# PJLab-ADG/DetZero

Measured on AMD Instinct MI355X. Metric: LiDAR frames/sec (160k pts, 0.1m voxels), higher is better.
Workload: dtype f32 as f16 pairs (hi+lo, 22-bit significand; 3 f16 MFMA per product, f32 accumulate)

## Files before the change

### detzero_amd/det_modules.py

```python
import contextlib
import os
from functools import partial

import numpy as np
import torch
import torch.nn as nn

from . import ops
from .lib import DetZeroHipError

PACKED_TABLES = bool(os.environ.get('DZ_TUNE_PACKED_TABLES'))

K3, S1, P1 = (3, 3, 3), (1, 1, 1), (1, 1, 1)


def _inference_only(module):
    if module.training:
        raise DetZeroHipError('%s: only the inference path is implemented on the HIP backend '
                              '(call .eval()); training is out of scope' % type(module).__name__)


def fold_bn(bn, conv_bias=None):
    w = bn.weight.detach().double()
    b = bn.bias.detach().double()
# ... 526 lines not shown


def bordered_zeros(name, shape, dev):
    ws = _WORKSPACE[0]
    if ws is None:
        return torch.zeros(shape, dtype=torch.float32, device=dev)
    key = (name, tuple(shape), str(dev))
    buf = ws.get(key)
    if buf is None:
        buf = ws[key] = torch.zeros(shape, dtype=torch.float32, device=dev)
    return buf


def nchw_to_padded_nhwc(x, pad=1):
    b, c, h, w = x.shape
    out = x.new_zeros((b, h + 2 * pad, w + 2 * pad, c))
    out[:, pad:pad + h, pad:pad + w, :] = x.permute(0, 2, 3, 1)
    return out


def _recode(img, enc, math, e_src=0, e_dst=0):
    if ops.storage_math(enc) == ops.storage_math(math) and e_src == e_dst:
        return img
    plain = ops.pair16_to_f32(img, enc) if enc else img
    if e_src != e_dst:
        plain = plain * (2.0 ** (e_dst - e_src))
    return ops.pair16_from_f32(plain, math=math) if math else plain


SKIP_EMPTY_TILES = os.environ.get('DZ_TUNE_SKIP_EMPTY_TILES', '1') != '0'
SPARSE_BEV_INPUT = os.environ.get('DZ_TUNE_SPARSE_BEV', '1') != '0'
FIRST_BLOCK_WIDE_GROUPS = os.environ.get('DZ_TUNE_FIRST_BLOCK_WIDE', '1') != '0'
FUSED_DEBLOCK_PHASES = os.environ.get('DZ_TUNE_DEBLOCK_PHASES', '1') != '0'


def conv_layer(inp, in_shape, w, scale, shift, relu, out, out_shape, *, cin, in_cstride, in_coff=0, ksize=3,
               stride=1, in_off=0, out_cstride, out_coff=0, out_s=1, out_d=(0, 0), groups=1, cout_pad=None,
               g_cout=None, g_ooff=None, ho=None, wo=None, batch=1, math=0, out_f32=False, phase_groups=False, in_rowidx=None,
               in_row_channels=0, in_rows=0, in_tiles=None):
    if cout_pad is None:
        cout_pad = w.shape[-2] if math else w.shape[-1]
    ops.conv2d(dict(
        inp=inp.data_ptr(), out=out.data_ptr(), w=w.data_ptr(),
        scale=scale.data_ptr() if scale is not None else None,
        shift=shift.data_ptr() if shift is not None else None,
        batch=batch, ho=ho, wo=wo, in_hp=in_shape[0], in_wp=in_shape[1], in_cstride=in_cstride, in_coff=in_coff,
        cin=cin, kh=ksize, kw=ksize, stride=stride, in_off=in_off,
        out_hp=out_shape[0], out_wp=out_shape[1], out_cstride=out_cstride, out_coff=out_coff,
        out_sy=out_s, out_sx=out_s, out_dy=out_d[0], out_dx=out_d[1],
        groups=groups, cout_pad=cout_pad,
        g_cout=g_cout if g_cout is not None else [cout_pad], g_ooff=g_ooff if g_ooff is not None else [0],
        relu=1 if relu else 0, phase_groups=1 if phase_groups else 0,
        in_rowidx=in_rowidx.data_ptr() if in_rowidx is not None else None, in_row_channels=int(in_row_channels), in_rows=int(in_rows),
        in_tiles=in_tiles.data_ptr() if in_tiles is not None else None),
        math=math, out_f32=out_f32, tiles=in_tiles)


class BaseBEVBackbone(_Cached):

    def __init__(self, model_cfg, input_channels):
        super().__init__()
        self.model_cfg = model_cfg
        layer_nums = list(model_cfg.LAYER_NUMS)
        layer_strides = list(model_cfg.LAYER_STRIDES)
        num_filters = list(model_cfg.NUM_FILTERS)
        upsample_strides = list(model_cfg.UPSAMPLE_STRIDES)
        num_upsample_filters = list(model_cfg.NUM_UPSAMPLE_FILTERS)
        assert len(layer_nums) == len(layer_strides) == len(num_filters) == len(upsample_strides)
        c_in_list = [input_channels, *num_filters[:-1]]
        self.blocks = nn.ModuleList()
        self.deblocks = nn.ModuleList()
        for idx in range(len(layer_nums)):
            cur = [nn.ZeroPad2d(1),
                   nn.Conv2d(c_in_list[idx], num_filters[idx], kernel_size=3, stride=layer_strides[idx], padding=0, bias=False),
                   nn.BatchNorm2d(num_filters[idx], eps=1e-3, momentum=0.01), nn.ReLU()]
            for _ in range(layer_nums[idx]):
                cur.extend([nn.Conv2d(num_filters[idx], num_filters[idx], kernel_size=3, padding=1, bias=False),
                            nn.BatchNorm2d(num_filters[idx], eps=1e-3, momentum=0.01), nn.ReLU()])
            self.blocks.append(nn.Sequential(*cur))
            s = upsample_strides[idx]
            if not (isinstance(s, int) and s >= 1):
                raise DetZeroHipError('BaseBEVBackbone: only integer UPSAMPLE_STRIDES >= 1 are supported')
            self.deblocks.append(nn.Sequential(
                nn.ConvTranspose2d(num_filters[idx], num_upsample_filters[idx], s, stride=s, bias=False),
                nn.BatchNorm2d(num_upsample_filters[idx], eps=1e-3, momentum=0.01), nn.ReLU()))
        self.num_bev_features = sum(num_upsample_filters)
        self.layer_strides, self.upsample_strides = layer_strides, upsample_strides
        self.num_filters, self.num_upsample_filters = num_filters, num_upsample_filters
# ... 75 lines not shown
                if not getattr(self, '_warned_capture_nl1', False):
                    self._warned_capture_nl1 = True
                    import warnings
                    warnings.warn('BaseBEVBackbone: graph capture of a %d-frame pass without an eager pass of the same size before it - empty tiles '
                                  'are skipped at the first layer only (run one eager pass first to skip them in all six)' % batch)
            tiles = ops.bev_tile_list(sparse_in[1], xh, xw, nl)
            zero = self._zero_response(lvl, xh, xw, sparse_in[0].shape[1], dev, batch) if nl > 1 else None
        for ci, cv in enumerate(convs):
            s = cv['stride']
            oh, ow = (xh + 2 - 3) // s + 1, (xw + 2 - 3) // s + 1
            if bufs is None:
                bufs = [bordered_zeros('bev2d.l%d.%d' % (li, k), (batch, oh + 2, ow + 2, cv['cout']), dev) for k in range(2)]
            y = out_last if (out_last is not None and ci == len(convs) - 1) else bufs[ci % 2]
            if sparse_in is not None and li == 0 and ci == 0:
                rows, ridx = sparse_in
                wz, scz, shz = self._p(cv, e_in, e_mid, key='w_zmajor')
                conv_layer(rows, (xh + 2, xw + 2), wz, scz, shz, True, y, (oh + 2, ow + 2),
                           cin=cv['cin'], in_cstride=xc, ksize=3, stride=s, in_off=0, out_cstride=cv['cout'],
                           out_d=(1, 1), ho=oh, wo=ow, batch=batch, math=self.math, in_rowidx=ridx, in_row_channels=rows.shape[1],
                           in_rows=rows.shape[0], in_tiles=tiles[0] if tiles is not None else None)
                if tiles is not None:
                    ops.bev_fill_empty_tiles(tiles[0], batch, oh, ow, shz, True, cv['cout'], y, self.math)
            else:
                tl = tiles[ci] if (tiles is not None and ci < tiles.shape[0]) else None
                wc, scc, shc = self._p(cv, e_in if (li == 0 and ci == 0) else e_mid, e_mid)
                conv_layer(x, (xh + 2, xw + 2), wc, scc, shc, True, y, (oh + 2, ow + 2),
                           cin=cv['cin'], in_cstride=xc, ksize=3, stride=s, in_off=0, out_cstride=cv['cout'],
                           out_d=(1, 1), ho=oh, wo=ow, batch=batch, math=self.math, in_tiles=tl)
                if tl is not None:
                    ops.bev_fill_empty_tiles(tl, batch, oh, ow, shc, True, cv['cout'], y, self.math, zero_resp=zero[ci])
            x, xh, xw, xc = y, oh, ow, cv['cout']
        return x, xh, xw, xc

    def _level_deblock(self, lvl, x, xh, xw, xc, concat, coff, h, w, batch):
        de = lvl['de']
        s = de['s']
        ctot = self.num_bev_features
        e_mid = self._e('spatial_features_2d')
        if xh * s != h or xw * s != w:
            raise DetZeroHipError('BaseBEVBackbone: deblock output %dx%d does not match %dx%d' % (xh * s, xw * s, h, w))
        if self.math and 1 < s * s <= 8 and FUSED_DEBLOCK_PHASES:
            conv_layer(x, (xh + 2, xw + 2), *self._p(de, e_mid, e_mid, key='w_phases'), True, concat,
                       (h + 2, w + 2), cin=de['cin'], in_cstride=xc, ksize=1, stride=1, in_off=1,
                       out_cstride=ctot, out_coff=coff, out_s=s, out_d=(1, 1), ho=xh, wo=xw, batch=batch, math=self.math,
                       groups=s * s, g_cout=[de['cout']] * (s * s), g_ooff=[0] * (s * s), phase_groups=True)
            return coff + de['cout']
        for dy in range(s):
            for dx in range(s):
                conv_layer(x, (xh + 2, xw + 2), *self._p(de['phases'][dy][dx], e_mid, e_mid, scale=de['scale'], shift=de['shift']), True, concat,
                           (h + 2, w + 2), cin=de['cin'], in_cstride=xc, ksize=1, stride=1, in_off=1,
                           out_cstride=ctot, out_coff=coff, out_s=s, out_d=(dy + 1, dx + 1), ho=xh, wo=xw,
                           batch=batch, math=self.math)
        return coff + de['cout']

    def run(self, bev, batch, sparse_in=None):
        plan = self.plan()
        if sparse_in is not None:
            rows, ridx = sparse_in
            dev = rows.device
            h, w = ridx.shape[1] - 2, ridx.shape[2] - 2
        else:
            dev = bev.device
            h, w = bev.shape[1] - 2, bev.shape[2] - 2
        concat = bordered_zeros('bev2d.concat', (batch, h + 2, w + 2, self.num_bev_features), dev)
        x, xh, xw, xc = bev, h, w, (bev.shape[3] if sparse_in is None else 2 * rows.shape[1])
        coff = 0
        for li, lvl in enumerate(plan):
            x, xh, xw, xc = self._level_convs(li, lvl, x, xh, xw, xc, batch, dev, sparse_in=sparse_in if li == 0 else None)
            coff = self._level_deblock(lvl, x, xh, xw, xc, concat, coff, h, w, batch)
        return concat

    def grouped_fits(self, nb, h, w):
        plan = self.plan()
        xh, xw, worst = h, w, 0
        for lvl in plan:
            s = lvl['convs'][0]['stride']
            xh, xw = (xh + 2 - 3) // s + 1, (xw + 2 - 3) // s + 1
            worst = max(worst, (xh + 2) * (xw + 2) * lvl['convs'][-1]['cout'] * 4)
        return nb * worst < 2 ** 31

    def run_grouped(self, nb, group, consume, bev=None, sparse_in=None):
        plan = self.plan()
        if sparse_in is not None:
            rows, ridx = sparse_in
            dev = rows.device
            h, w = ridx.shape[1] - 2, ridx.shape[2] - 2
            cin0 = 2 * rows.shape[1]
        else:
            dev = bev.device
            h, w = bev.shape[1] - 2, bev.shape[2] - 2
            cin0 = bev.shape[3]
        l0 = plan[0]
        s0 = l0['convs'][0]['stride']
        h0, w0 = (h + 2 - 3) // s0 + 1, (w + 2 - 3) // s0 + 1
        c0 = l0['convs'][-1]['cout']
        if len(l0['convs']) < 2:
            raise DetZeroHipError('BaseBEVBackbone.run_grouped: the first block needs at least two convolutions')
        x0_all = bordered_zeros('bev2d.x0_all', (nb, h0 + 2, w0 + 2, c0), dev)
        widest = max([cin0] + [cv['cout'] for cv in l0['convs']])
        group1 = max(group, min(nb, (2 ** 31 - 1) // ((h + 2) * (w + 2) * widest * 4))) if FIRST_BLOCK_WIDE_GROUPS else group
        for g0 in range(0, nb, group1):
            ng = min(group1, nb - g0)
            sp = (rows, ridx[g0:g0 + ng]) if sparse_in is not None else None
            self._level_convs(0, l0, None if sp is not None else bev[g0:g0 + ng], h, w, cin0, ng, dev, sparse_in=sp, out_last=x0_all[g0:g0 + ng])
        outs = [(x0_all, h0, w0, c0)]
        x, xh, xw, xc = outs[0]
        for li in range(1, len(plan)):
            x, xh, xw, xc = self._level_convs(li, plan[li], x, xh, xw, xc, nb, dev)
            outs.append((x, xh, xw, xc))
        for g0 in range(0, nb, group):
            ng = min(group, nb - g0)
            concat = bordered_zeros('bev2d.concat', (ng, h + 2, w + 2, self.num_bev_features), dev)
            coff = 0
            for lvl, (x, xh, xw, xc) in zip(plan, outs):
                coff = self._level_deblock(lvl, x[g0:g0 + ng], xh, xw, xc, concat, coff, h, w, ng)
            consume(concat, g0, ng)

    def forward(self, data_dict):
        _inference_only(self)
        with torch.no_grad():
            bev = data_dict.get('_nhwc_spatial_features', None)
            enc = data_dict.get('_nhwc_math', 0)
            e_src = int(data_dict.get('_nhwc_exp', 0) or 0)
            if bev is None:
                bev, enc = nchw_to_padded_nhwc(data_dict['spatial_features'].float()), 0
                e_src = 0
            bev = _recode(bev, enc, self.math, e_src, self._e('encoded'))
            concat = self.run(bev, bev.shape[0])
        e_out = self._e('spatial_features_2d')
        data_dict['_nhwc_spatial_features_2d'] = concat
        data_dict['_nhwc_math'] = self.math
        data_dict['_nhwc_exp'] = e_out
        plain = ops.pair16_to_f32(concat, self.math) if self.math else concat
        if e_out:
            plain = plain * (2.0 ** -e_out)
        data_dict['spatial_features_2d'] = plain[:, 1:-1, 1:-1, :].permute(0, 3, 1, 2)
        return data_dict


class SeparateHead(nn.Module):

    def __init__(self, input_channels, sep_head_dict, init_bias=-2.19, use_bias=False):
        super().__init__()
        self.sep_head_dict = sep_head_dict
        for cur_name in self.sep_head_dict:
            output_channels = self.sep_head_dict[cur_name]['out_channels']
            num_conv = self.sep_head_dict[cur_name]['num_conv']
            fc_list = []
# ... 230 lines not shown
```

### detzero_amd/lib.py

```python
import ctypes
import os

import torch

_HERE = os.path.dirname(os.path.abspath(__file__))
LIB_PATH = os.path.join(_HERE, 'libdetzero_hip.so')


ERR_INVALID, ERR_WORKSPACE, ERR_HIP, ERR_UNSUPPORTED = -1, -2, -3, -4


class DetZeroHipError(RuntimeError):
    pass


c_int, c_float, c_size_t, c_void_p, c_double = ctypes.c_int, ctypes.c_float, ctypes.c_size_t, ctypes.c_void_p, ctypes.c_double
_I3 = c_int * 3
_F3 = c_float * 3
_F6 = c_float * 6
_I8 = c_int * 8


class Conv2dDesc(ctypes.Structure):
    _fields_ = [
# ... 75 lines not shown
    'dz_spconv_forward_split_packed': (c_int, [c_void_p, c_int, c_int, c_void_p, c_void_p, c_int, c_void_p, c_void_p, c_void_p,
                                               c_void_p, c_void_p, c_int, c_void_p, c_int, c_int, c_void_p]),
    'dz_spconv_tile_rows': (c_int, []),
    'dz_spconv_tile_info_words': (c_int, []),
    'dz_spconv_tile_table_entries': (c_int, []),
    'dz_build_tiles_halo_stride': (c_size_t, [c_int]),
    'dz_build_tiles': (c_int, [c_void_p, c_int, c_int, c_void_p, c_void_p, c_void_p, c_void_p, c_void_p, c_void_p]),
    'dz_spconv_tiles_forward': (c_int, [c_void_p, c_int, c_int, c_void_p, c_void_p, c_void_p, c_void_p, c_int, c_int, c_void_p, c_void_p,
                                        c_void_p, c_void_p, c_void_p, c_int, c_void_p, c_int, c_int, c_void_p]),
    'dz_spconv_tiles_variant': (ctypes.c_char_p, [c_int, c_int]),
    'dz_spconv_x_tile_rows': (c_int, [c_int, c_int]),
    'dz_spconv_x_window_rows': (c_int, [c_int, c_int]),
    'dz_spconv_x_windows_words': (c_size_t, [c_int, c_int]),
    'dz_spconv_x_windows': (c_int, [c_void_p, c_int, c_void_p, c_int, c_void_p, c_void_p, c_void_p, c_void_p]),
    'dz_build_neighbors_packed_x': (c_int, [c_void_p, c_void_p, c_int, c_void_p, c_void_p, c_int, c_int, c_int, c_int, c_void_p, c_void_p, c_int,
                                            c_void_p, c_void_p, c_void_p, c_void_p]),
    'dz_spconv_forward_split_x': (c_int, [c_void_p, c_int, c_int, c_void_p, c_void_p, c_void_p, c_int, c_int, c_void_p, c_void_p, c_void_p, c_void_p,
                                          c_void_p, c_int, c_void_p, c_int, c_int, c_void_p]),
    'dz_spconv_x_variant': (ctypes.c_char_p, [c_int, c_int]),
    'dz_spconv_forward_x_f32': (c_int, [c_void_p, c_int, c_int, c_void_p, c_void_p, c_void_p, c_int, c_int, c_void_p, c_void_p, c_void_p, c_void_p,
                                        c_void_p, c_int, c_void_p, c_int, c_void_p]),
    'dz_spconv_x_f32_window_rows': (c_int, [c_int, c_int]),
    'dz_spconv_x_f32_variant': (ctypes.c_char_p, [c_int, c_int]),
    'dz_bev_tile_list_words': (c_size_t, [c_int, c_int, c_int]),
    'dz_bev_tile_list': (c_int, [c_void_p, c_int, c_int, c_int, c_int, c_int, c_int, c_void_p, c_void_p, c_void_p]),
    'dz_bev_fill_empty_tiles': (c_int, [c_void_p, c_int, c_int, c_int, c_void_p, c_int, c_int, c_void_p, c_int, c_int, c_int, c_int, c_void_p, c_int, c_void_p]),
    'dz_bev_row_index': (c_int, [c_void_p, c_void_p, c_int, c_int, c_int, c_int, c_int, c_int, c_int, c_void_p, c_void_p]),
    'dz_sparse_to_bev_split': (c_int, [c_void_p, c_void_p, c_void_p, c_int, c_int, c_int, c_int, c_int, c_int, c_void_p,
                                       c_void_p]),
    'dz_sparse_to_bev_split_dense': (c_int, [c_void_p, c_int, c_void_p, c_void_p, c_int, c_int, c_int, c_int, c_int, c_int, c_int, c_void_p,
                                             c_void_p]),
    'dz_conv2d_forward_split': (c_int, [ctypes.POINTER(Conv2dDesc), c_int, c_int, c_void_p]),
    'dz_conv2d_variant_split': (ctypes.c_char_p, [ctypes.POINTER(Conv2dDesc), c_int]),
    'dz_spconv_variant_split': (ctypes.c_char_p, [c_int, c_int]),
    'dz_spconv_variant_split_arm': (ctypes.c_char_p, [c_int, c_int, c_int, c_int, c_size_t]),
    'dz_spconv_variant_split_packed': (ctypes.c_char_p, [c_int, c_int]),
    'dz_xattn_folded_supported': (c_int, [c_int, c_int, c_int]),
    'dz_xattn_folded_workspace_bytes': (ctypes.c_size_t, [c_int, c_int]),
    'dz_xattn_folded': (c_int, [c_void_p] * 6 + [c_int] * 5 + [ctypes.c_float, c_void_p, ctypes.c_size_t, c_void_p, c_void_p]),
    'dz_roi_bev_features': (c_int, [c_void_p, c_int, c_void_p, ctypes.c_long, ctypes.c_long, c_int, c_int, c_int] + [ctypes.c_float] * 4 + [c_int, c_void_p, c_void_p]),
    'dz_linear_splitk_workspace_bytes': (ctypes.c_size_t, [c_int, c_int, c_int]),
    'dz_linear_forward_splitk': (c_int, [c_void_p, c_int, c_int, c_int, c_void_p, c_int, c_int, c_void_p, c_void_p, c_int, c_void_p, c_int, c_int, c_void_p,
                                         ctypes.c_size_t, c_void_p]),
    'dz_mha_core_split': (c_int, [c_void_p, c_void_p, c_void_p, c_void_p, c_int, c_int, c_int, c_int, ctypes.c_float, c_void_p, c_int, c_void_p]),
    'dz_pdv_sa_pool_supported': (c_int, [c_int] * 7),
    'dz_pdv_sa_pool': (c_int, [c_void_p, c_int, c_int, c_void_p, c_void_p, c_int, c_void_p, c_void_p, c_int, c_void_p, c_void_p, c_int,
                               c_void_p, c_int, c_void_p, c_void_p, c_int, c_void_p, c_int, c_void_p, c_void_p, c_int, c_int, c_void_p, c_void_p]),
    'dz_pdv_encoder_front': (c_int, [c_void_p, c_int, c_void_p, c_void_p, ctypes.c_long] + [c_void_p] * 9 + [c_int, c_void_p]),
    'dz_pdv_encoder_back': (c_int, [c_void_p, c_void_p, c_void_p, c_void_p, ctypes.c_long, c_void_p, c_void_p, c_void_p, c_void_p, c_float, c_void_p, c_void_p,
                                    c_void_p, c_void_p, c_void_p, c_void_p, c_float, c_void_p, c_int, c_int, c_void_p]),
    'dz_self_attention_split_supported': (c_int, [c_int, c_int]),
    'dz_self_attention_split': (c_int, [c_void_p, c_void_p, c_void_p, c_int, c_int, c_int, c_void_p, c_int, c_void_p]),
    'dz_pdv_sa_pool_split_supported': (c_int, [c_int] * 7),
    'dz_pdv_sa_pool_split': (c_int, [c_void_p, c_int, c_int, c_void_p, c_void_p, ctypes.c_long, c_int, c_void_p, c_void_p, c_int, c_void_p, c_void_p, c_int,
                                     c_void_p, c_int, c_void_p, c_void_p, c_int, c_void_p, c_int, c_void_p, c_void_p, c_int, c_int, c_int, c_void_p, c_int, c_void_p]),
    'dz_mlp_chain_forward': (c_int, [c_void_p, ctypes.c_long, c_void_p, c_void_p, c_void_p, c_void_p, c_int, c_int] + [c_void_p] * 10 + [c_int, c_void_p]),
    'dz_pointnet3_forward': (c_int, [c_void_p, ctypes.c_long] + [c_void_p] * 9 + [c_int, c_int, c_void_p, c_void_p, c_int, c_int, c_void_p]),
    'dz_centerhead_decode_workspace_bytes': (c_size_t, [c_int] * 4),
    'dz_centerhead_decode': (c_int, [c_void_p, c_int, c_int, c_int, c_int, c_int, c_float, c_void_p, c_void_p,
                                     c_void_p, c_int, c_int, c_void_p, c_void_p, c_void_p, c_void_p, c_void_p,
                                     c_size_t, c_void_p]),
    'dz_nms_workspace_bytes': (c_size_t, [c_int]),
    'dz_nms_rotated': (c_int, [c_void_p, c_void_p, c_int, c_float, c_int, c_void_p, c_void_p, c_void_p, c_size_t,
                               c_void_p]),
    'dz_nms_rotated_batched': (c_int, [c_void_p, c_void_p, c_int, c_int, c_float, c_int, c_void_p, c_void_p, c_void_p, c_size_t,
                                       c_void_p]),
# ... 92 lines not shown
```

### detzero_amd/ops.py

```python
import ctypes
import os

import numpy as np
import torch

from . import lib as L


def _dev():
    return torch.device('cuda', torch.cuda.current_device())


def _ws(nbytes):
    return torch.empty((max(int(nbytes), 256),), dtype=torch.uint8, device=_dev())


def grid_size_of(pc_range, voxel_size):
    r = np.asarray(pc_range, dtype=np.float32)
    return np.round((r[3:6] - r[0:3]) / np.array(voxel_size)).astype(np.int64)


def voxelize_hard_nosync(points, pc_range, voxel_size, max_points, max_voxels, xy_range_mask=False):
    lib = L.load()
    L.require_cuda(points)
# ... 474 lines not shown
    for _ in red:
        up = up.unsqueeze(-2)
    return w.float() * up, down


def level_rows_f32(rows, level, math=0):
    plain = pair16_to_f32(rows, math) if math else rows
    e = int(getattr(level, 'act_exp', 0) or 0)
    return plain * (2.0 ** -e) if e else plain


def pair16_from_f32(x, c_dst=None, math=1):
    lib = L.load()
    L.require_cuda(x)
    x = x.contiguous()
    c = x.shape[-1]
    c_dst = c if c_dst is None else c_dst
    rows = x.numel() // c
    out = torch.empty((*x.shape[:-1], c_dst), dtype=torch.float32, device=x.device)
    L.check(lib.dz_pair16_from_f32(L.ptr(x), rows, c, c_dst, storage_math(math), L.ptr(out), L.stream()), 'dz_pair16_from_f32')
    return out


def pair16_to_f32(x, math=1):
    lib = L.load()
    L.require_cuda(x)
    x = x.contiguous()
    c = x.shape[-1]
    out = torch.empty_like(x)
    L.check(lib.dz_pair16_to_f32(L.ptr(x), x.numel() // c, c, storage_math(math), L.ptr(out), L.stream()), 'dz_pair16_to_f32')
    return out


def conv2d(desc_kwargs, math=0, out_f32=False, tiles=None):
    lib = L.load()
    d = L.Conv2dDesc()
    g_cout = desc_kwargs.pop('g_cout')
    g_ooff = desc_kwargs.pop('g_ooff')
    for k, v in desc_kwargs.items():
        setattr(d, k, v)
    for i, v in enumerate(g_cout):
        d.g_cout[i] = int(v)
    for i, v in enumerate(g_ooff):
        d.g_ooff[i] = int(v)

    def launch():
        if math:
            L.check(lib.dz_conv2d_forward_split(ctypes.byref(d), int(math), 1 if out_f32 else 0, L.stream()), 'dz_conv2d_forward_split')
        else:
            L.check(lib.dz_conv2d_forward(ctypes.byref(d), L.stream()), 'dz_conv2d_forward')
    if PROFILER is None:
        launch()
        return
    m = d.batch * d.ho * d.wo
    taps = d.kh * d.kw
    cout = sum(d.g_cout[i] for i in range(d.groups))
    flops = 2.0 * m * taps * d.cin * cout
    nbytes = 4.0 * (m * d.cin * (1 if d.phase_groups else d.groups) + m * cout + taps * d.cin * d.cout_pad * d.groups)
    if tiles is not None:
        n_run, n_skip = (int(v) for v in tiles[:2].tolist())
        share = n_run / float(max(n_run + n_skip, 1))
        flops *= share
        nbytes = 4.0 * (share * (m * d.cin + m * cout) + taps * d.cin * d.cout_pad * d.groups)
    name = (lib.dz_conv2d_variant_split(ctypes.byref(d), 1 if out_f32 else 0) if math else lib.dz_conv2d_variant(ctypes.byref(d))).decode()
    PROFILER.wrap(name, flops, nbytes, launch)


def linear(x, w, scale, shift, relu, cout, out=None, group_shift=None, group_rows=0):
    lib = L.load()
    L.require_cuda(x, w, scale, shift, group_shift)
    rows, cin = x.shape
    cout_pad = w.shape[1]
    if out is None:
        out = torch.empty((rows, cout), dtype=torch.float32, device=x.device)
    rc = lib.dz_linear_forward(L.ptr(x), rows, cin, x.stride(0), L.ptr(w), cout, cout_pad, L.ptr(scale),
                               L.ptr(shift), L.ptr(group_shift), int(group_rows), 1 if relu else 0, L.ptr(out),
                               out.stride(0), L.stream())
    L.check(rc, 'dz_linear_forward')
    return out


SPLITK_MAX_ROWS, SPLITK_MIN_CIN = 2048, 4096


def linear_splitk_ok(rows, cin):
    return 0 < rows <= SPLITK_MAX_ROWS and cin >= SPLITK_MIN_CIN and cin % 256 == 0


def linear_splitk(x, w, scale, shift, relu, cout, splits=8):
    lib = L.load()
    L.require_cuda(x, w, scale, shift)
    rows, cin = x.shape
    cout_pad = w.shape[1]
    nbytes = lib.dz_linear_splitk_workspace_bytes(rows, cout_pad, splits)
    ws = torch.empty(((nbytes + 3) // 4,), dtype=torch.float32, device=x.device)
    out = torch.empty((rows, cout), dtype=torch.float32, device=x.device)
    rc = lib.dz_linear_forward_splitk(L.ptr(x), rows, cin, x.stride(0), L.ptr(w), cout, cout_pad, L.ptr(scale), L.ptr(shift), 1 if relu else 0, L.ptr(out),
                                      out.stride(0), int(splits), L.ptr(ws), nbytes, L.stream())
# ... 316 lines not shown
```

### include/detzero_hip.h

```cpp
#ifndef DETZERO_HIP_H
#define DETZERO_HIP_H

#include <stddef.h>
#include <stdint.h>

#ifdef __cplusplus
extern "C" {
#endif

#define DZ_OK 0
#define DZ_ERR_INVALID (-1)
#define DZ_ERR_WORKSPACE (-2)
#define DZ_ERR_HIP (-3)
#define DZ_ERR_UNSUPPORTED (-4)

const char *dz_version(void);
const char *dz_last_error(void);
int dz_device_cu_count(void);


size_t dz_voxelize_hard_workspace_bytes(int n, int gx, int gy, int gz, int max_points);
int dz_voxelize_hard(const float *points, int n, int c, const float *h_range6, const float *h_vsize3,
                     const int *h_grid3, int xy_range_mask, int max_points, int max_voxels, float *voxels,
                     int *coords_zyx, int *num_points, int *d_num_voxels, void *ws, size_t ws_bytes,
// ... 105 lines not shown
const char *dz_spconv_tiles_variant(int cin, int cout);
int dz_spconv_forward_split_packed(const float *in, int in_rows, int cin, const int *nbr_packed, const uint32_t *tile_masks,
                                   int cap_out, const int *d_m_out, const float *w, const float *scale, const float *shift,
                                   const float *residual, int relu, float *out, int cout, int math, void *stream);
int dz_spconv_x_tile_rows(int cin, int cout);
int dz_spconv_x_window_rows(int cin, int cout);
size_t dz_spconv_x_windows_words(int cap_out, int tile_rows);
int dz_spconv_x_windows(const int *nbr_packed, int cap_out, const int *d_m_out, int tile_rows, int *windows, int *nbr_sorted, int *perm,
                        void *stream);
int dz_build_neighbors_packed_x(const int *coords, const int *d_m, int cap, const uint32_t *bitmap, const uint32_t *prefix, int b, int d,
                                int h, int w, int *nbr_packed, uint32_t *tile_masks, int tile_rows, int *windows, int *nbr_sorted,
                                int *perm, void *stream);
int dz_spconv_forward_split_x(const float *in, int in_rows, int cin, const int *nbr_packed, const int *perm, int *windows, int tile_rows,
                              int cap_out, const int *d_m_out, const float *w, const float *scale, const float *shift,
                              const float *residual, int relu, float *out, int cout, int math, void *stream);
const char *dz_spconv_x_variant(int cin, int cout);
int dz_spconv_forward_x_f32(const float *in, int in_rows, int cin, const int *nbr_packed, const int *perm, int *windows, int tile_rows,
                            int cap_out, const int *d_m_out, const float *w, const float *scale, const float *shift,
                            const float *residual, int relu, float *out, int cout, void *stream);
int dz_spconv_x_f32_window_rows(int cin, int cout);
const char *dz_spconv_x_f32_variant(int cin, int cout);
int dz_bev_row_index(const uint32_t *bitmap, const uint32_t *prefix, int batch, int d, int h, int w, int layout, int pad, int feat_rows,
                     int *idx, void *stream);
size_t dz_bev_tile_list_words(int batch, int ho, int wo);
int dz_bev_tile_list(const int *idx, int batch, int hp, int wp, int ho, int wo, int nlists, int *lists, unsigned char *mind_ws, void *stream);
int dz_bev_fill_empty_tiles(const int *list, int batch, int ho, int wo, const float *shift, int relu, int cout, float *out, int out_hp, int out_wp,
                            int out_cstride, int out_coff, const float *zero_resp, int math, void *stream);
int dz_sparse_to_bev_split(const float *feats, const int *coords, const int *d_m, int cap, int c, int d, int h,
                           int w, int pad, float *bev, void *stream);
int dz_sparse_to_bev_split_dense(const float *feats, int feat_rows, const uint32_t *bitmap, const uint32_t *prefix, int batch, int c,
                                 int d, int h, int w, int layout, int pad, float *bev, void *stream);
int dz_conv2d_forward_split(const dz_conv2d_desc *h_desc, int math, int out_f32, void *stream);
const char *dz_conv2d_variant_split(const dz_conv2d_desc *h_desc, int out_f32);
int dz_linear_forward_split(const float *x, long rows, int cin, int x_stride, const float *w, int cout, int cout_pad, const float *scale,
                            const float *shift, const float *group_shift, int group_rows, int relu, float *y, int y_stride, int math,
                            int out_f32, int group_max, void *stream);
const char *dz_spconv_variant_split(int cin, int cout);
const char *dz_spconv_variant_split_arm(int cin, int cout, int kvol, int has_tile_masks, size_t nbr_bytes);
const char *dz_spconv_variant_split_packed(int cin, int cout);
int dz_xattn_folded_supported(int lq, int e, int heads);
size_t dz_xattn_folded_workspace_bytes(int b, int lk);
int dz_xattn_folded(const float *q, const float *mem, const uint8_t *key_padding_mask, const float *wk_oi, const float *wv_io, const float *bv,
                    int b, int lq, int lk, int e, int heads, float scale, float *workspace, size_t workspace_bytes, float *out, void *stream);
int dz_mlp_chain_forward(const float *x, long rows, const float *wa, const float *sa, const float *ba, const float *group_shift, int ldg, int group_rows,
                         const float *wb, const float *sb, const float *bb, const float *wk, const float *bk, const float *wv, const float *bv,
                         float *mem, float *k, float *v, int math, void *stream);
int dz_pointnet3_forward(const float *x, long rows, const float *w1, const float *s1, const float *b1, const float *w2, const float *s2,
                         const float *b2, const float *w3, const float *s3, const float *b3, int c3, int group_rows, float *tap, float *out,
                         int x_cols_f32, int math, void *stream);

size_t dz_centerhead_decode_workspace_bytes(int batch, int hw, int ncls, int k);
int dz_centerhead_decode(const float *head, int batch, int h, int w, int ncls, int k, float score_thresh,
                         const float *h_limit6, const float *h_range6, const float *h_vsize3, int stride,
                         int use_iou, float *boxes, float *scores, int *labels, int *d_counts, void *ws,
                         size_t ws_bytes, void *stream);

int dz_roi_bev_features(const float *boxes, int n, const float *bev, long row_stride, long pix_stride, int h, int w, int c, float x_lo, float y_lo,
                        float voxel_x, float voxel_y, int stride, float *out, void *stream);

size_t dz_nms_workspace_bytes(int n_cap);
int dz_nms_rotated(const float *boxes, const int *d_n, int n_cap, float thresh, int post_max, int *keep,
                   int *d_num_keep, void *ws, size_t ws_bytes, void *stream);
int dz_nms_rotated_batched(const float *boxes, const int *d_n, int batch, int n_cap, float thresh, int post_max,
                           int *keep, int *d_num_keep, void *ws, size_t ws_bytes, void *stream);
int dz_pack_detections(const float *boxes, const float *scores, const int *labels, const int *keep,
                       const int *d_num_keep, int batch, int k, int post_max, float *out, void *stream);
// ... 122 lines not shown
```

Baseline: 1129.

## Fuse all BEV deblock levels into one persistent multi-level kernel

Adds a HIP kernel that runs the 1x1 transposed-conv deblocks of every backbone level and phase in one launch. Work is split into (level, phase) classes, and spare blocks per XCD are handed out in proportion to estimated cost. Each block keeps its weights in registers and double-buffers input pixel tiles through LDS. The aim is to cut per-level launch overhead and the tail idle time of small levels, at the cost of a large LDS footprint and a restricted set of supported shapes, with fallback to the old per-level path.

```diff
diff --git a/detzero_amd/csrc/deblock_h.hip b/detzero_amd/csrc/deblock_h.hip
--- /dev/null
+++ b/detzero_amd/csrc/deblock_h.hip
@@ -0,0 +1,270 @@
+#include "hgemm.h"
+
+namespace dz {
+
+constexpr int DB_NT = 512;
+constexpr int DB_COUT = 256;
+constexpr int DB_TILE_WORDS = 8192;
+constexpr int DB_MAX_LEVELS = 4, DB_MAX_CLASSES = 32;
+
+template <int K>
+struct DbTile {
+    static constexpr int BP = DB_TILE_WORDS / K, PT = BP / 32, CT = 1, THREADS = DB_NT;
+    static constexpr int ROW_U4 = K / 4 + 1;
+    static constexpr int PPR = K / 4;
+    static constexpr int PIECES = BP * PPR / DB_NT;
+    static constexpr int LDS_BYTES = DB_NT / 64 * STG_WAVE_BYTES;
+    static_assert(PIECES == 4 && BP % 32 == 0, "a pixel tile is four 16-byte pieces per thread");
+};
+constexpr int DB_BUF_U4 = 2112;
+constexpr int DB_MAX_BP = 64;
+constexpr int DB_LDS_STG = 2 * DB_BUF_U4 * 16;
+constexpr int DB_LDS_SC = DB_LDS_STG + DB_NT / 64 * STG_WAVE_BYTES;
+constexpr int DB_LDS_PIX = DB_LDS_SC + 2 * DB_COUT * 4;
+constexpr int DB_LDS_BYTES = DB_LDS_PIX + 2 * DB_MAX_BP * 4;
+static_assert(DB_LDS_BYTES <= 160 * 1024, "does not fit the LDS of a CU");
+
+struct DbLevel {
+    const float *in, *w, *scale, *shift;
+    float *out;
+    int m_total, ho, wo;
+    int in_hp, in_wp, in_cstride, in_coff, in_off, cin;
+    int out_hp, out_wp, out_cstride, out_coff, out_sy, out_sx, out_dy, out_dx;
+    int relu;
+};
+struct DbClass { short level, phase, first, n; };
+struct DbArgs {
+    DbLevel lv[DB_MAX_LEVELS];
+    DbClass cls[DB_MAX_CLASSES];
+    int n_classes;
+};
+
+template <class M, int K>
+__device__ __forceinline__ void deblock_run(const DbLevel &L, int phase, int xcd, int j, int nj, unsigned char *smem_raw) {
+    using T = DbTile<K>;
+    constexpr int BP = T::BP, PT = T::PT, ROW_U4 = T::ROW_U4, PPR = T::PPR, KS = K / 16;
+    v4u *const buf = reinterpret_cast<v4u *>(smem_raw);
+    float *const sc_s = reinterpret_cast<float *>(smem_raw + DB_LDS_SC), *const sh_s = sc_s + DB_COUT;
+    int *const out_pix = reinterpret_cast<int *>(smem_raw + DB_LDS_PIX);
+
+    const int tid = threadIdx.x, lane = tid & 63, wid = tid >> 6, h = lane >> 5;
+    const int ntiles = (L.m_total + BP - 1) / BP;
+    const int per_xcd = (ntiles + 7) >> 3;
+    const int band_hi = min(ntiles, (xcd + 1) * per_xcd);
+    int tile = xcd * per_xcd + j;
+    if (tile >= band_hi) return;
+
+    v4u w_hi[KS], w_lo[KS];
+    {
+        const v4u *wr = reinterpret_cast<const v4u *>(L.w) + ((size_t)phase * DB_COUT + wid * 32 + (lane & 31)) * PPR + h * 2;
+#pragma unroll
+        for (int q = 0; q < KS; ++q) {
+            w_hi[q] = wr[q * 4];
+            w_lo[q] = wr[q * 4 + 1];
+        }
+    }
+    if (tid < DB_COUT) {
+        sc_s[tid] = L.scale ? L.scale[tid] : 1.f;
+        sh_s[tid] = L.shift ? L.shift[tid] : 0.f;
+    }
+    const int ph_dy = phase / L.out_sx, ph_dx = phase % L.out_sx;
+    const int prow = tid / PPR, pu = tid % PPR;
+    const v4u *const in_u4 = reinterpret_cast<const v4u *>(L.in) + (L.in_coff >> 2) + pu;
+    const unsigned int in_row_u4 = (unsigned int)L.in_cstride >> 2;
+
+    auto issue = [&](int t, v4u (&st)[4]) {
+#pragma unroll
+        for (int i = 0; i < 4; ++i) {
+            const unsigned int m = (unsigned int)min(t * BP + prow + i * (DB_NT / PPR), L.m_total - 1);
+            const unsigned int x = m % (unsigned int)L.wo, ty = m / (unsigned int)L.wo;
+            const unsigned int y = ty % (unsigned int)L.ho, b = ty / (unsigned int)L.ho;
+            const unsigned int ip = (b * L.in_hp + y + L.in_off) * L.in_wp + x + L.in_off;
+            st[i] = in_u4[(size_t)ip * in_row_u4];
+        }
+    };
+    auto store = [&](const v4u (&st)[4], int par, int t) {
+        v4u *const d = buf + par * DB_BUF_U4 + prow * ROW_U4 + pu;
+#pragma unroll
+        for (int i = 0; i < 4; ++i) d[i * (DB_NT / PPR) * ROW_U4] = st[i];
+        if (tid < BP) {
+            const int m = t * BP + tid;
+            int op = -1;
+            if (m < L.m_total) {
+                const unsigned int x = (unsigned int)m % (unsigned int)L.wo, ty = (unsigned int)m / (unsigned int)L.wo;
+                const unsigned int y = ty % (unsigned int)L.ho, b = ty / (unsigned int)L.ho;
+                op = (int)((b * L.out_hp + y * L.out_sy + L.out_dy + ph_dy) * L.out_wp + x * L.out_sx + L.out_dx + ph_dx);
+            }
+            out_pix[par * DB_MAX_BP + tid] = op;
+        }
+    };
+
+    v4u st[4];
+    issue(tile, st);
+    store(st, 0, tile);
+    bool has_next = tile + nj < band_hi;
+    if (has_next) issue(tile + nj, st);
+    __syncthreads();
+
+    const int poff = (lane & 31) * ROW_U4 + h * 2;
+    const bool relu = L.relu != 0;
+    unsigned char *const out_b = reinterpret_cast<unsigned char *>(L.out);
+    int par = 0;
+    for (;;) {
+        f32x16 acc[1][PT];
+#pragma unroll
+        for (int pt = 0; pt < PT; ++pt)
+#pragma unroll
+            for (int e = 0; e < 16; ++e) acc[0][pt][e] = 0.f;
+        const v4u *const pb = buf + par * DB_BUF_U4 + poff;
+#pragma unroll
+        for (int q = 0; q < KS; ++q) {
+#pragma unroll
+            for (int pt = 0; pt < PT; ++pt) {
+                const v4u p_hi = pb[pt * 32 * ROW_U4 + q * 4];
+                if constexpr (M::TERMS == 1) {
+                    acc[0][pt] = M::mma(w_hi[q], p_hi, acc[0][pt]);
+                } else {
+                    const v4u p_lo = pb[pt * 32 * ROW_U4 + q * 4 + 1];
+                    acc[0][pt] = M::mma(w_lo[q], p_hi, acc[0][pt]);
+                    acc[0][pt] = M::mma(w_hi[q], p_lo, acc[0][pt]);
+                    acc[0][pt] = M::mma(w_hi[q], p_hi, acc[0][pt]);
+                }
+            }
+        }
+        const bool has_next2 = has_next && tile + 2 * nj < band_hi;
+        if (has_next) {
+            store(st, par ^ 1, tile + nj);
+            if (has_next2) issue(tile + 2 * nj, st);
+        }
+        const int *const opx = out_pix + par * DB_MAX_BP;
+        store_tile_pair16<T, M>(acc, smem_raw + DB_LDS_STG, sc_s, sh_s, 0, DB_COUT, relu, nullptr, out_b, 0, wid, lane, wid, [&](int lr) {
+            const int op = opx[lr];
+            return op >= 0 ? ((size_t)op * L.out_cstride + L.out_coff) * 4 : ~size_t(0);
+        });
+        if (!has_next) break;
+        __syncthreads();
+        tile += nj;
+        par ^= 1;
+        has_next = has_next2;
+    }
+}
+
+template <class M>
+__global__ __launch_bounds__(DB_NT) void k_deblock_h(DbArgs a) {
+    extern __shared__ __attribute__((aligned(16))) unsigned char smem_raw[];
+    const int xcd = blockIdx.x & 7, jloc = blockIdx.x >> 3;
+    int level = -1, phase = 0, j = 0, nj = 1;
+#pragma unroll
+    for (int i = 0; i < DB_MAX_CLASSES; ++i) {
+        if (i < a.n_classes && jloc >= a.cls[i].first && jloc < a.cls[i].first + a.cls[i].n) {
+            level = a.cls[i].level; phase = a.cls[i].phase; j = jloc - a.cls[i].first; nj = a.cls[i].n;
+        }
+    }
+    if (level < 0) return;
+    DbLevel L = a.lv[0];
+#pragma unroll
+    for (int i = 1; i < DB_MAX_LEVELS; ++i)
+        if (level == i) L = a.lv[i];
+    if (L.cin == 128) deblock_run<M, 128>(L, phase, xcd, j, nj, smem_raw);
+    else deblock_run<M, 256>(L, phase, xcd, j, nj, smem_raw);
+}
+
+static const char *deblocks_refusal(const dz_conv2d_desc *lv, int n_levels) {
+    if (!lv || n_levels < 1 || n_levels > DB_MAX_LEVELS) return "1 to 4 levels";
+    int classes = 0;
+    for (int i = 0; i < n_levels; ++i) {
+        const dz_conv2d_desc &d = lv[i];
+        if (!d.in || !d.out || !d.w) return "null pointer";
+        if (d.kh != 1 || d.kw != 1 || d.stride != 1) return "1x1 kernels with stride 1 only";
+        if (d.cin != 128 && d.cin != 256) return "cin must be 128 or 256";
+        if (d.cout_pad != DB_COUT) return "cout must be 256";
+        if (d.group_shift || d.group_max || d.in_rowidx || d.in_tiles) return "group_shift / group_max / in_rowidx / in_tiles are not supported";
+        if (d.out_sy < 1 || d.out_sx < 1 || d.out_sy * d.out_sx > 8) return "at most 8 phases (s x s <= 8)";
+        if (d.groups != (d.phase_groups ? d.out_sy * d.out_sx : 1)) return "groups must be the out_sy x out_sx phases (phase_groups) or 1";
+        for (int g = 0; g < d.groups; ++g)
+            if (d.g_cout[g] != DB_COUT || d.g_ooff[g] != 0) return "every phase writes all 256 channels at out_coff";
+        if (d.in_cstride % 8 || d.in_coff % 8 || d.out_cstride % 8 || d.out_coff % 8) return "channel strides / offsets in multiples of 8";
+        if (d.in_coff < 0 || d.in_coff + d.cin > d.in_cstride || d.out_coff < 0 || d.out_coff + DB_COUT > d.out_cstride) return "channel slice leaves the pixel row";
+        if (d.batch < 0 || d.ho < 0 || d.wo < 0 || d.in_off < 0) return "negative extent";
+        if ((long)d.batch * d.ho * d.wo > 0) {
+            if (d.ho - 1 + d.in_off >= d.in_hp || d.wo - 1 + d.in_off >= d.in_wp) return "input pixels leave the input image";
+            const int ph_y = d.phase_groups ? d.out_sy - 1 : 0, ph_x = d.phase_groups ? d.out_sx - 1 : 0;
+            if (d.out_dy < 0 || d.out_dx < 0 || (d.ho - 1) * d.out_sy + d.out_dy + ph_y >= d.out_hp || (d.wo - 1) * d.out_sx + d.out_dx + ph_x >= d.out_wp)
+                return "output leaves the output image";
+            if ((size_t)d.batch * d.in_hp * d.in_wp * d.in_cstride * sizeof(float) >= 0x80000000ull ||
+                (size_t)d.batch * d.out_hp * d.out_wp >= 0x80000000ull)
+                return "image exceeds the 2 GiB buffer window";
+            classes += d.groups;
+        }
+    }
+    if (classes > DB_MAX_CLASSES) return "too many (level, phase) classes";
+    return nullptr;
+}
+
+static bool math_is_split(int math) { return math == DZ_MATH_F16X2 || math == DZ_MATH_BF16X2 || math == DZ_MATH_F16; }
+
+}
+
+using namespace dz;
+
+extern "C" {
+
+int dz_bev_deblocks_supported(const dz_conv2d_desc *levels, int n_levels, int math) {
+    return math_is_split(math) && !deblocks_refusal(levels, n_levels) ? 1 : 0;
+}
+
+const char *dz_bev_deblocks_variant(const dz_conv2d_desc *levels, int n_levels, int math) {
+    return dz_bev_deblocks_supported(levels, n_levels, math) ? "k_deblock_h<8x32xK>" : "none";
+}
+
+int dz_bev_deblocks_forward_split(const dz_conv2d_desc *levels, int n_levels, int math, void *stream_) {
+    hipStream_t stream = (hipStream_t)stream_;
+    DZ_CHECK_ARG(math_is_split(math), "dz_bev_deblocks_forward_split: math %d is not a split mode", math);
+    if (const char *why = deblocks_refusal(levels, n_levels)) {
+        set_error("dz_bev_deblocks_forward_split: %s", why);
+        return DZ_ERR_UNSUPPORTED;
+    }
+    DbArgs a = {};
+    double cost[DB_MAX_CLASSES];
+    int nc = 0;
+    for (int i = 0; i < n_levels; ++i) {
+        const dz_conv2d_desc &d = levels[i];
+        DbLevel &L = a.lv[i];
+        L.in = d.in; L.w = d.w; L.scale = d.scale; L.shift = d.shift; L.out = d.out;
+        L.m_total = (int)((long)d.batch * d.ho * d.wo); L.ho = d.ho; L.wo = d.wo;
+        L.in_hp = d.in_hp; L.in_wp = d.in_wp; L.in_cstride = d.in_cstride; L.in_coff = d.in_coff; L.in_off = d.in_off; L.cin = d.cin;
+        L.out_hp = d.out_hp; L.out_wp = d.out_wp; L.out_cstride = d.out_cstride; L.out_coff = d.out_coff;
+        L.out_sy = d.out_sy; L.out_sx = d.out_sx; L.out_dy = d.out_dy; L.out_dx = d.out_dx; L.relu = d.relu;
+        if (L.m_total == 0) continue;
+        const int bp = DB_TILE_WORDS / d.cin;
+        const double c = (double)ceil_div(L.m_total, bp) * (bp / 32) * (3.0 * d.cin / 16 + 9.0);
+        for (int g = 0; g < d.groups; ++g) {
+            a.cls[nc].level = (short)i; a.cls[nc].phase = (short)g; a.cls[nc].n = 1;
+            cost[nc++] = c;
+        }
+    }
+    if (nc == 0) return DZ_OK;
+    int per_xcd = device_cus() / 8;
+    if (per_xcd < nc) per_xcd = nc;
+    for (int spare = per_xcd - nc; spare > 0; --spare) {
+        int best = 0;
+        for (int c = 1; c < nc; ++c)
+            if (cost[c] / a.cls[c].n > cost[best] / a.cls[best].n) best = c;
+        ++a.cls[best].n;
+    }
+    for (int c = 0, first = 0; c < nc; ++c) { a.cls[c].first = (short)first; first += a.cls[c].n; }
+    a.n_classes = nc;
+    auto launch = [&](auto m_t) -> int {
+        using M = typename decltype(m_t)::type;
+        static PerDeviceFlags lds_done;
+        if (int rc_ = reserve_lds(reinterpret_cast<const void *>(&k_deblock_h<M>), DB_LDS_BYTES, lds_done, "dz_bev_deblocks_forward_split")) return rc_;
+        hipLaunchKernelGGL((k_deblock_h<M>), dim3(8u * per_xcd), dim3(DB_NT), DB_LDS_BYTES, stream, a);
+        DZ_LAUNCH_CHECK();
+        return DZ_OK;
+    };
+    if (math == DZ_MATH_F16X2) return launch(TypeTag<MathF16>{});
+    if (math == DZ_MATH_F16) return launch(TypeTag<MathF16H>{});
+    return launch(TypeTag<MathBF16>{});
+}
+
+}
diff --git a/detzero_amd/det_modules.py b/detzero_amd/det_modules.py
--- a/detzero_amd/det_modules.py
+++ b/detzero_amd/det_modules.py
@@ -582,15 +582,16 @@
 SPARSE_BEV_INPUT = os.environ.get('DZ_TUNE_SPARSE_BEV', '1') != '0'
 FIRST_BLOCK_WIDE_GROUPS = os.environ.get('DZ_TUNE_FIRST_BLOCK_WIDE', '1') != '0'
 FUSED_DEBLOCK_PHASES = os.environ.get('DZ_TUNE_DEBLOCK_PHASES', '1') != '0'
-
-
-def conv_layer(inp, in_shape, w, scale, shift, relu, out, out_shape, *, cin, in_cstride, in_coff=0, ksize=3,
-               stride=1, in_off=0, out_cstride, out_coff=0, out_s=1, out_d=(0, 0), groups=1, cout_pad=None,
-               g_cout=None, g_ooff=None, ho=None, wo=None, batch=1, math=0, out_f32=False, phase_groups=False, in_rowidx=None,
-               in_row_channels=0, in_rows=0, in_tiles=None):
+DEBLOCK_STREAM = os.environ.get('DZ_TUNE_DEBLOCK_STREAM', '1') != '0'
+
+
+def conv_desc(inp, in_shape, w, scale, shift, relu, out, out_shape, *, cin, in_cstride, in_coff=0, ksize=3,
+              stride=1, in_off=0, out_cstride, out_coff=0, out_s=1, out_d=(0, 0), groups=1, cout_pad=None,
+              g_cout=None, g_ooff=None, ho=None, wo=None, batch=1, math=0, phase_groups=False, in_rowidx=None,
+              in_row_channels=0, in_rows=0, in_tiles=None):
     if cout_pad is None:
         cout_pad = w.shape[-2] if math else w.shape[-1]
-    ops.conv2d(dict(
+    return dict(
         inp=inp.data_ptr(), out=out.data_ptr(), w=w.data_ptr(),
         scale=scale.data_ptr() if scale is not None else None,
         shift=shift.data_ptr() if shift is not None else None,
@@ -602,8 +603,11 @@
         g_cout=g_cout if g_cout is not None else [cout_pad], g_ooff=g_ooff if g_ooff is not None else [0],
         relu=1 if relu else 0, phase_groups=1 if phase_groups else 0,
         in_rowidx=in_rowidx.data_ptr() if in_rowidx is not None else None, in_row_channels=int(in_row_channels), in_rows=int(in_rows),
-        in_tiles=in_tiles.data_ptr() if in_tiles is not None else None),
-        math=math, out_f32=out_f32, tiles=in_tiles)
+        in_tiles=in_tiles.data_ptr() if in_tiles is not None else None)
+
+
+def conv_layer(*args, math=0, out_f32=False, in_tiles=None, **kw):
+    ops.conv2d(conv_desc(*args, math=math, in_tiles=in_tiles, **kw), math=math, out_f32=out_f32, tiles=in_tiles)
 
 
 class BaseBEVBackbone(_Cached):
@@ -745,18 +749,30 @@
             x, xh, xw, xc = y, oh, ow, cv['cout']
         return x, xh, xw, xc
 
+    def _deblock_desc(self, lvl, x, xh, xw, xc, concat, coff, h, w, batch):
+        de = lvl['de']
+        s = de['s']
+        e_mid = self._e('spatial_features_2d')
+        if xh * s != h or xw * s != w:
+            raise DetZeroHipError('BaseBEVBackbone: deblock output %dx%d does not match %dx%d' % (xh * s, xw * s, h, w))
+        common = dict(cin=de['cin'], in_cstride=xc, ksize=1, stride=1, in_off=1, out_cstride=self.num_bev_features, out_coff=coff, out_s=s,
+                      out_d=(1, 1), ho=xh, wo=xw, batch=batch, math=self.math)
+        if self.math and 1 < s * s <= 8 and FUSED_DEBLOCK_PHASES:
+            return conv_desc(x, (xh + 2, xw + 2), *self._p(de, e_mid, e_mid, key='w_phases'), True, concat, (h + 2, w + 2),
+                             groups=s * s, g_cout=[de['cout']] * (s * s), g_ooff=[0] * (s * s), phase_groups=True, **common)
+        if self.math and s == 1:
+            return conv_desc(x, (xh + 2, xw + 2), *self._p(de['phases'][0][0], e_mid, e_mid, scale=de['scale'], shift=de['shift']), True, concat,
+                             (h + 2, w + 2), **common)
+        return None
+
     def _level_deblock(self, lvl, x, xh, xw, xc, concat, coff, h, w, batch):
         de = lvl['de']
         s = de['s']
         ctot = self.num_bev_features
         e_mid = self._e('spatial_features_2d')
-        if xh * s != h or xw * s != w:
-            raise DetZeroHipError('BaseBEVBackbone: deblock output %dx%d does not match %dx%d' % (xh * s, xw * s, h, w))
-        if self.math and 1 < s * s <= 8 and FUSED_DEBLOCK_PHASES:
-            conv_layer(x, (xh + 2, xw + 2), *self._p(de, e_mid, e_mid, key='w_phases'), True, concat,
-                       (h + 2, w + 2), cin=de['cin'], in_cstride=xc, ksize=1, stride=1, in_off=1,
-                       out_cstride=ctot, out_coff=coff, out_s=s, out_d=(1, 1), ho=xh, wo=xw, batch=batch, math=self.math,
-                       groups=s * s, g_cout=[de['cout']] * (s * s), g_ooff=[0] * (s * s), phase_groups=True)
+        desc = self._deblock_desc(lvl, x, xh, xw, xc, concat, coff, h, w, batch)
+        if desc is not None:
+            ops.conv2d(desc, math=self.math)
             return coff + de['cout']
         for dy in range(s):
             for dx in range(s):
@@ -765,6 +781,19 @@
                            out_cstride=ctot, out_coff=coff, out_s=s, out_d=(dy + 1, dx + 1), ho=xh, wo=xw,
                            batch=batch, math=self.math)
         return coff + de['cout']
+
+    def _deblocks(self, plan, outs, g0, ng, concat, h, w):
+        if self.math and DEBLOCK_STREAM:
+            descs, coff = [], 0
+            for lvl, (x, xh, xw, xc) in zip(plan, outs):
+                descs.append(self._deblock_desc(lvl, x[g0:g0 + ng], xh, xw, xc, concat, coff, h, w, ng))
+                coff += lvl['de']['cout']
+            if all(d is not None for d in descs) and ops.bev_deblocks_supported(descs, self.math):
+                ops.bev_deblocks(descs, self.math)
+                return
+        coff = 0
+        for lvl, (x, xh, xw, xc) in zip(plan, outs):
+            coff = self._level_deblock(lvl, x[g0:g0 + ng], xh, xw, xc, concat, coff, h, w, ng)
 
     def run(self, bev, batch, sparse_in=None):
         plan = self.plan()
@@ -777,10 +806,11 @@
             h, w = bev.shape[1] - 2, bev.shape[2] - 2
         concat = bordered_zeros('bev2d.concat', (batch, h + 2, w + 2, self.num_bev_features), dev)
         x, xh, xw, xc = bev, h, w, (bev.shape[3] if sparse_in is None else 2 * rows.shape[1])
-        coff = 0
+        outs = []
         for li, lvl in enumerate(plan):
             x, xh, xw, xc = self._level_convs(li, lvl, x, xh, xw, xc, batch, dev, sparse_in=sparse_in if li == 0 else None)
-            coff = self._level_deblock(lvl, x, xh, xw, xc, concat, coff, h, w, batch)
+            outs.append((x, xh, xw, xc))
+        self._deblocks(plan, outs, 0, batch, concat, h, w)
         return concat
 
     def grouped_fits(self, nb, h, w):
@@ -824,9 +854,7 @@
         for g0 in range(0, nb, group):
             ng = min(group, nb - g0)
             concat = bordered_zeros('bev2d.concat', (ng, h + 2, w + 2, self.num_bev_features), dev)
-            coff = 0
-            for lvl, (x, xh, xw, xc) in zip(plan, outs):
-                coff = self._level_deblock(lvl, x[g0:g0 + ng], xh, xw, xc, concat, coff, h, w, ng)
+            self._deblocks(plan, outs, g0, ng, concat, h, w)
             consume(concat, g0, ng)
 
     def forward(self, data_dict):
diff --git a/detzero_amd/lib.py b/detzero_amd/lib.py
--- a/detzero_amd/lib.py
+++ b/detzero_amd/lib.py
@@ -131,6 +131,9 @@
                                              c_void_p]),
     'dz_conv2d_forward_split': (c_int, [ctypes.POINTER(Conv2dDesc), c_int, c_int, c_void_p]),
     'dz_conv2d_variant_split': (ctypes.c_char_p, [ctypes.POINTER(Conv2dDesc), c_int]),
+    'dz_bev_deblocks_supported': (c_int, [ctypes.POINTER(Conv2dDesc), c_int, c_int]),
+    'dz_bev_deblocks_forward_split': (c_int, [ctypes.POINTER(Conv2dDesc), c_int, c_int, c_void_p]),
+    'dz_bev_deblocks_variant': (ctypes.c_char_p, [ctypes.POINTER(Conv2dDesc), c_int, c_int]),
     'dz_spconv_variant_split': (ctypes.c_char_p, [c_int, c_int]),
     'dz_spconv_variant_split_arm': (ctypes.c_char_p, [c_int, c_int, c_int, c_int, c_size_t]),
     'dz_spconv_variant_split_packed': (ctypes.c_char_p, [c_int, c_int]),
diff --git a/detzero_amd/ops.py b/detzero_amd/ops.py
--- a/detzero_amd/ops.py
+++ b/detzero_amd/ops.py
@@ -530,17 +530,30 @@
     return out
 
 
+def _conv2d_desc(desc_kwargs):
+    d = L.Conv2dDesc()
+    for k, v in desc_kwargs.items():
+        if k in ('g_cout', 'g_ooff'):
+            arr = getattr(d, k)
+            for i, e in enumerate(v):
+                arr[i] = int(e)
+        else:
+            setattr(d, k, v)
+    return d
+
+
+def _conv2d_work(d):
+    m = d.batch * d.ho * d.wo
+    taps = d.kh * d.kw
+    cout = sum(d.g_cout[i] for i in range(d.groups))
+    flops = 2.0 * m * taps * d.cin * cout
+    nbytes = 4.0 * (m * d.cin * (1 if d.phase_groups else d.groups) + m * cout + taps * d.cin * d.cout_pad * d.groups)
+    return flops, nbytes
+
+
 def conv2d(desc_kwargs, math=0, out_f32=False, tiles=None):
     lib = L.load()
-    d = L.Conv2dDesc()
-    g_cout = desc_kwargs.pop('g_cout')
-    g_ooff = desc_kwargs.pop('g_ooff')
-    for k, v in desc_kwargs.items():
-        setattr(d, k, v)
-    for i, v in enumerate(g_cout):
-        d.g_cout[i] = int(v)
-    for i, v in enumerate(g_ooff):
-        d.g_ooff[i] = int(v)
+    d = _conv2d_desc(desc_kwargs)
 
     def launch():
         if math:
@@ -550,18 +563,38 @@
     if PROFILER is None:
         launch()
         return
-    m = d.batch * d.ho * d.wo
-    taps = d.kh * d.kw
-    cout = sum(d.g_cout[i] for i in range(d.groups))
-    flops = 2.0 * m * taps * d.cin * cout
-    nbytes = 4.0 * (m * d.cin * (1 if d.phase_groups else d.groups) + m * cout + taps * d.cin * d.cout_pad * d.groups)
+    flops, nbytes = _conv2d_work(d)
     if tiles is not None:
+        m = d.batch * d.ho * d.wo
+        taps = d.kh * d.kw
+        cout = sum(d.g_cout[i] for i in range(d.groups))
         n_run, n_skip = (int(v) for v in tiles[:2].tolist())
         share = n_run / float(max(n_run + n_skip, 1))
         flops *= share
         nbytes = 4.0 * (share * (m * d.cin + m * cout) + taps * d.cin * d.cout_pad * d.groups)
     name = (lib.dz_conv2d_variant_split(ctypes.byref(d), 1 if out_f32 else 0) if math else lib.dz_conv2d_variant(ctypes.byref(d))).decode()
     PROFILER.wrap(name, flops, nbytes, launch)
+
+
+def _deblock_descs(descs):
+    return (L.Conv2dDesc * len(descs))(*[_conv2d_desc(k) for k in descs])
+
+
+def bev_deblocks_supported(descs, math):
+    return 0 < len(descs) <= 4 and bool(L.load().dz_bev_deblocks_supported(_deblock_descs(descs), len(descs), int(math)))
+
+
+def bev_deblocks(descs, math):
+    lib = L.load()
+    arr = _deblock_descs(descs)
+
+    def launch():
+        L.check(lib.dz_bev_deblocks_forward_split(arr, len(descs), int(math), L.stream()), 'dz_bev_deblocks_forward_split')
+    if PROFILER is None:
+        launch()
+        return
+    work = [_conv2d_work(d) for d in arr]
+    PROFILER.wrap(lib.dz_bev_deblocks_variant(arr, len(descs), int(math)).decode(), sum(w[0] for w in work), sum(w[1] for w in work), launch)
 
 
 def linear(x, w, scale, shift, relu, cout, out=None, group_shift=None, group_rows=0):
diff --git a/include/detzero_hip.h b/include/detzero_hip.h
--- a/include/detzero_hip.h
+++ b/include/detzero_hip.h
@@ -161,6 +161,9 @@
                                  int d, int h, int w, int layout, int pad, float *bev, void *stream);
 int dz_conv2d_forward_split(const dz_conv2d_desc *h_desc, int math, int out_f32, void *stream);
 const char *dz_conv2d_variant_split(const dz_conv2d_desc *h_desc, int out_f32);
+int dz_bev_deblocks_supported(const dz_conv2d_desc *h_levels, int n_levels, int math);
+int dz_bev_deblocks_forward_split(const dz_conv2d_desc *h_levels, int n_levels, int math, void *stream);
+const char *dz_bev_deblocks_variant(const dz_conv2d_desc *h_levels, int n_levels, int math);
 int dz_linear_forward_split(const float *x, long rows, int cin, int x_stride, const float *w, int cout, int cout_pad, const float *scale,
                             const float *shift, const float *group_shift, int group_rows, int relu, float *y, int y_stride, int math,
                             int out_f32, int group_max, void *stream);
```

Result: no change. 1139, median of 6 (+0.8%).
